# croci/bluest

Measured on AMD Instinct MI355X. Metric: Phi-assemblies/s, higher is better.
Workload: dtype f64; 1 GPU; n=20 models, groups up to size 5 (K_tot=21699), n_out=8, Wishart covariances; one step = V and grad V of one allocation for all outputs; n_models=20, k_max=5, K_tot=21699, n_out=8, batch=1, parallelism=single GPU, evaluation=stored group inverses, launch=hipGraph replay of 20-step graphs (20 of 20 steps), rest eager

## Files before the change

### bluest_amd/build.py

```python
import os
import shutil
import subprocess
import sys

HERE = os.path.dirname(os.path.abspath(__file__))
ROOT = os.path.dirname(HERE)
CSRC = os.path.join(HERE, "csrc")
SOURCES = ["runtime.hip", "mirrors.hip", "plan.hip", "spg.hip", "intproj.hip", "xchg.hip", "newton.hip", "matfree.hip", "mfmc.hip", "mlmc.hip", "covproj.hip", "pilot.hip", "gsums.hip", "fields.hip", "moments.hip", "pilot4.hip", "field_moments.hip", "wave_probe.hip"]
HEADERS = ["common.hpp", "solve.hpp", "plan.hpp", "spg_state.hpp", "jacobi.hpp", "subset_search.hpp", "staging.hpp"]
OBJDIR = os.path.join(CSRC, "_build")
HDR = os.path.join(ROOT, "include", "bluest_hip.h")
LIB = os.path.join(HERE, "libbluest_hip.so")
ARCH = "gfx950"


def hipcc():
    for cand in (os.environ.get("HIPCC"), shutil.which("hipcc"), "/opt/rocm/bin/hipcc"):
        if cand and os.path.exists(cand):
            return cand
    raise RuntimeError("hipcc not found (looked at $HIPCC, PATH, /opt/rocm/bin/hipcc)")


def _inputs():
    return [os.path.join(CSRC, f) for f in SOURCES + HEADERS] + [HDR]


STAMP = os.path.join(OBJDIR, "hipcc_flags.txt")


def _extra_flags():
    return os.environ.get("BLUEST_EXTRA_HIPCC_FLAGS", "").split()


def up_to_date():
    if not os.path.exists(LIB) or os.path.getmtime(LIB) < max(os.path.getmtime(f) for f in _inputs()):
        return False
    try:
        built_with = open(STAMP).read().split()
    except OSError:
        built_with = []
    return built_with == _extra_flags()


SHIM_SRC = os.path.join(HERE, "csrc", "cmisc_shim.cpp")


def shim_path():
    import sysconfig
    return os.path.join(HERE, "shim", "_cmisc_bluest" + sysconfig.get_config_var("EXT_SUFFIX"))


def build_shim(force=False, verbose=False):
    out = shim_path()
    if not force and os.path.exists(out) and os.path.getmtime(out) >= max(os.path.getmtime(SHIM_SRC), os.path.getmtime(HDR)):
        return out
    import pybind11
    import sysconfig
    os.makedirs(os.path.dirname(out), exist_ok=True)
    cmd = ["g++", "-O2", "-shared", "-std=c++17", "-fPIC", "-I" + pybind11.get_include(), "-I" + sysconfig.get_paths()["include"],
           "-I" + os.path.join(ROOT, "include"), SHIM_SRC, "-o", out, "-L" + HERE, "-lbluest_hip", "-Wl,-rpath,$ORIGIN/.."]
    if verbose:
        print(" ".join(cmd))
    subprocess.check_call(cmd)
    return out


def build(force=False, verbose=False):
    if not force and up_to_date():
        build_shim(force=False, verbose=verbose)
        return LIB
    from concurrent.futures import ThreadPoolExecutor
    os.makedirs(OBJDIR, exist_ok=True)
    flags = ["--offload-arch=" + ARCH, "-O3", "-std=c++17", "-fPIC", "-pthread", "-I" + os.path.join(ROOT, "include"),
             "-I" + CSRC] + _extra_flags()

    def compile_one(name):
        obj = os.path.join(OBJDIR, os.path.splitext(name)[0] + ".o")
        cmd = [hipcc()] + flags + ["-c", os.path.join(CSRC, name), "-o", obj]
        if verbose:
            print(" ".join(cmd))
        subprocess.check_call(cmd)
        return obj

    with ThreadPoolExecutor(max_workers=min(len(SOURCES), os.cpu_count() or 1)) as pool:
        objs = list(pool.map(compile_one, SOURCES))
    cmd = [hipcc(), "--offload-arch=" + ARCH, "-shared", "-fPIC", "-pthread", "-o", LIB] + objs
    if verbose:
        print(" ".join(cmd))
    subprocess.check_call(cmd)
    with open(STAMP, "w") as f:
        f.write(" ".join(_extra_flags()))
    build_shim(force=True, verbose=verbose)
    return LIB


if __name__ == "__main__":
    print(build(force="--force" in sys.argv, verbose=True))
```

### bluest_amd/csrc/plan.hip

```cpp

#include "common.hpp"

static int g_debug_timing = getenv("BLUEST_DEBUG_TIMING") ? 1 : 0;
struct PhaseTimer {
    std::chrono::steady_clock::time_point t0 = std::chrono::steady_clock::now();
    const char *what;
    explicit PhaseTimer(const char *w) : what(w) {}
    void lap(const char *phase)
    {
        if (!g_debug_timing) return;
        const auto t1 = std::chrono::steady_clock::now();
        fprintf(stderr, "[bluest timing] %s: %s %.3f ms\n", what, phase, std::chrono::duration<double, std::milli>(t1 - t0).count());
        t0 = t1;
    }
};


#include "plan.hpp"
#include "spg_state.hpp"

template <typename COLT> __device__ __forceinline__ int4 load_cols4(const COLT *p);
template <> __device__ __forceinline__ int4 load_cols4<int32_t>(const int32_t *p) { return *reinterpret_cast<const int4 *>(p); }
template <> __device__ __forceinline__ int4 load_cols4<uint16_t>(const uint16_t *p)
{
    const uint2 w = *reinterpret_cast<const uint2 *>(p);
    return make_int4((int)(w.x & 0xffffu), (int)(w.x >> 16), (int)(w.y & 0xffffu), (int)(w.y >> 16));
}
__device__ __forceinline__ bool phi_gate_closed(const int32_t *gate) { return gate && uniform_word(gate) == 0; }
template <int WPB> __device__ __forceinline__ uint32_t phi_wave_chunk()
{
    if constexpr (WPB == 1) return blockIdx.x;
    else return blockIdx.x * WPB + (uint32_t)__builtin_amdgcn_readfirstlane((int)(threadIdx.x >> 6));
}
template <int WPB, typename COLT>
__global__ __launch_bounds__(64 * WPB) void k_phi_chunks(const double *__restrict__ vals, const COLT *__restrict__ cols,
                                                    int iters, int64_t n_chunks, const double *__restrict__ m,
                                                    int64_t m_stride, int n_cand, double2 *__restrict__ partial,
                                                    const int32_t *__restrict__ pslot, int64_t pstride,
                                                    const int32_t *__restrict__ gate)
{
    kernarg_now(vals, cols, iters, n_chunks, m, m_stride, n_cand, partial, pslot, pstride, gate);
    const bool closed = phi_gate_closed(gate);
    const uint32_t chunk = phi_wave_chunk<WPB>();
    const uint32_t lane = threadIdx.x & 63;
    if (closed) return;
    if (chunk >= (uint32_t)n_chunks) return;
    const int32_t slot_ld = *(pslot ? pslot + chunk : reinterpret_cast<const int32_t *>(cols));
    const uint64_t base = (uint64_t)chunk * ((uint32_t)iters * 256u);
    const char *vb = reinterpret_cast<const char *>(vals + base);
    const char *cb = reinterpret_cast<const char *>(cols + base);
    const double *mc = m;
    char *pc = reinterpret_cast<char *>(partial);
    for (int c = 0; c < n_cand; c++, mc += m_stride, pc += pstride * (int64_t)sizeof(double2)) {
        double s = 0.0, amax = 0.0;
        uint32_t vo = lane * 32u, co = lane * (uint32_t)(4 * sizeof(COLT));
        int it = 0;
        do {
            const double2 *vp = reinterpret_cast<const double2 *>(vb + vo);
            const double2 v01 = vp[0], v23 = vp[1];
            const int4 cc = load_cols4<COLT>(reinterpret_cast<const COLT *>(cb + co));
            const double m0 = mc[cc.x], m1 = mc[cc.y], m2 = mc[cc.z], m3 = mc[cc.w];
            s = fma(v01.x, m0, s);
            s = fma(v01.y, m1, s);
            s = fma(v23.x, m2, s);
            s = fma(v23.y, m3, s);
            amax = fmax(fmax(amax, fmax(fabs(m0), fabs(m1))), fmax(fabs(m2), fabs(m3)));
            vo += 2048u; co += (uint32_t)(256 * sizeof(COLT));
        } while (++it < iters);
        s = wave_sum_dpp(s);
        amax = wave_max_dpp(amax);
        const uint32_t slot = pslot ? (uint32_t)lane_value_here(slot_ld) : chunk;
        if (lane == 0) *reinterpret_cast<double2 *>(pc + slot * 16u) = make_double2(s, amax);
    }
}

template <int OB, int WPB, typename COLT>
__global__ __launch_bounds__(64 * WPB) void k_phi_chunks_shared(const double *__restrict__ vals, const COLT *__restrict__ cols,
                                                           int iters, int64_t ncpo, int n_out, const double *__restrict__ m,
                                                           int64_t m_stride, int n_cand, int64_t pstride, const int32_t *__restrict__ pslot,
                                                           int slots_per_output, double2 *__restrict__ partial, const int32_t *__restrict__ gate)
{
    kernarg_now(vals, cols, iters, ncpo, n_out, m, m_stride, n_cand, pstride, pslot, slots_per_output, partial, gate);
    const bool closed = phi_gate_closed(gate);
    const uint32_t chunk = phi_wave_chunk<WPB>();
    const uint32_t lane = threadIdx.x & 63;
    const uint32_t o0 = blockIdx.y * OB;
    if (closed) return;
    if (chunk >= (uint32_t)ncpo) return;
    const int32_t slot_ld = *(pslot ? pslot + chunk : reinterpret_cast<const int32_t *>(cols));
    const uint32_t ostride = pslot ? (uint32_t)slots_per_output : (uint32_t)ncpo;
    const uint32_t CH = (uint32_t)iters * 256u;
    const char *cb = reinterpret_cast<const char *>(cols + (uint64_t)chunk * CH);
    const uint64_t per_out = (uint64_t)(uint32_t)ncpo * CH;
    const char *vb[OB];
    vb[0] = reinterpret_cast<const char *>(vals + (uint64_t)(o0 * (uint32_t)ncpo + chunk) * CH);
#pragma unroll
    for (int oo = 1; oo < OB; oo++) vb[oo] = vb[oo - 1] + (o0 + oo < (uint32_t)n_out ? per_out * sizeof(double) : 0);
    constexpr int NR = wave_sum_multi_regs(OB);
    uint32_t po[NR];
    bool mine[NR];
#pragma unroll
    for (int j = 0; j < NR; j++) {
        const uint32_t o = o0 + wave_sum_multi_index<OB>(lane, j);
        mine[j] = wave_sum_multi_owner<OB>(lane) && o < (uint32_t)n_out;
        po[j] = o * ostride * 16u;
    }
    const double *mc = m;
    char *pc = reinterpret_cast<char *>(partial);
    for (int c = 0; c < n_cand; c++, mc += m_stride, pc += pstride * (int64_t)sizeof(double2)) {
        double s[OB];
#pragma unroll
        for (int oo = 0; oo < OB; oo++) s[oo] = 0.0;
        double amax = 0.0;
        uint32_t vo = lane * 32u, co = lane * (uint32_t)(4 * sizeof(COLT));
        int it = 0;
        do {
            const int4 cc = load_cols4<COLT>(reinterpret_cast<const COLT *>(cb + co));
            double2 v01[OB], v23[OB];
#pragma unroll
            for (int oo = 0; oo < OB; oo++) {
                const double2 *vp = reinterpret_cast<const double2 *>(vb[oo] + vo);
                v01[oo] = vp[0];
                v23[oo] = vp[1];
            }
            const double m0 = mc[cc.x], m1 = mc[cc.y], m2 = mc[cc.z], m3 = mc[cc.w];
            amax = fmax(fmax(amax, fmax(fabs(m0), fabs(m1))), fmax(fabs(m2), fabs(m3)));
#pragma unroll
            for (int oo = 0; oo < OB; oo++) {
                s[oo] = fma(v01[oo].x, m0, s[oo]);
                s[oo] = fma(v01[oo].y, m1, s[oo]);
                s[oo] = fma(v23[oo].x, m2, s[oo]);
                s[oo] = fma(v23[oo].y, m3, s[oo]);
            }
            vo += 2048u; co += (uint32_t)(256 * sizeof(COLT));
        } while (++it < iters);
        amax = wave_max_dpp(amax);
        double t[NR];
        wave_sum_multi<OB>(s, t);
        const uint32_t slot = pslot ? (uint32_t)lane_value_here(slot_ld) : chunk;
#pragma unroll
        for (int j = 0; j < NR; j++)
            if (mine[j]) *reinterpret_cast<double2 *>(pc + (po[j] + slot * 16u)) = make_double2(t[j], amax);
    }
}

__device__ __forceinline__ bool gate_closed(const int32_t *gate, int *s_closed)
{
    if (!gate) return false;
    if (threadIdx.x == 0) *s_closed = __hip_atomic_load(gate, __ATOMIC_RELAXED, __HIP_MEMORY_SCOPE_AGENT) == 0 ? 1 : 0;
    __syncthreads();
    return *s_closed != 0;
}

template <int NT>
__global__ __launch_bounds__(fold_threads(NT)) void k_solve_from_chunks(int N, int n_out, const RowDesc *__restrict__ rows, int nsym, FoldReg reg,
                                                           const double2 *__restrict__ partial, int64_t n_chunks,
                                                           double delta, int want_v, double *__restrict__ var,
                                                           double *__restrict__ v, int32_t *__restrict__ status,
                                                           const int32_t *__restrict__ gate, double *__restrict__ spg_state, int last_slot, int32_t *__restrict__ spg_enable,
                                                           unsigned int *__restrict__ ticket)
{
    __shared__ SolveLds<NT> lds;
    __shared__ double spg_ls[SPG_STATE_DOUBLES];
    __shared__ int s_closed;
    kernarg_now(N, n_out, rows, nsym, reg.Cd, reg.Co, reg.rank_ab, partial, n_chunks, gate, spg_state);
    const int o = blockIdx.x, c = blockIdx.y, tid = threadIdx.x;
    if (gate_closed(gate, &s_closed)) {
        if (spg_state && tid < WAVE && spg_closed_last(ticket + 16, gridDim.x * gridDim.y, tid))
            spg_decide_wave(spg_state, var, status, n_out, last_slot, spg_enable, spg_ls, tid);
        return;
    }
    SpgPrefetch pf;
    if (spg_state && tid < WAVE) spg_prefetch_state(spg_state, tid, pf);
    if (N < NT) { clear_pads(lds, N, tid, fold_threads(NT)); __syncthreads(); }
    fold_rows(lds, N, rows, o, nsym, partial + (int64_t)c * n_chunks, tid, fold_threads(NT), reg);
    __syncthreads();
    if (tid >= WAVE) return;
    const int lane = tid;
    if (spg_state) spg_prefetch_parts(pf, lane);
    const int64_t e = (int64_t)c * n_out + o;
    if (want_v & 2) {
        if (lane == 0) { var[e] = lds.at(0, 0); status[e] = 0; }
        return;
    }
    const double am = (lane < N) ? lds.amax[lane] : 0.0;
    const bool big = __ballot(am >= 0.05) != 0ull;
    const int reps = (want_v & 4) ? 2 : 1;
    double V_mine = 0.0;
    int32_t st_mine = 0;
    for (int rep = 0; rep < reps; rep++)
        solve_wave<NT>(lds, N, delta, am > 1.0e-6, am > 0.0, big, (want_v & 1) != 0, &V_mine, v + e * N, &st_mine, lane);
    if (lane == 0) { var[e] = V_mine; status[e] = st_mine; }
    if (spg_state) {
        int last = 0;
        if (n_out == 1) {
// ... 125 lines not shown
            const int sh = pow2_exponent(wave_max(rmax));
            if (lane < N)
                for (int j = 0; j < N; j++) A[lane * LD + j] = ldexp(A[lane * LD + j], -sh);
            wave_lds_sync();
            jacobi_pinv_lds(A, Q, N, LD, lane);
            const double w = lane < N ? A[lane * LD + lane] : 0.0;
            const double cut = 1.0e-15 * wave_max(fabs(w));
            if (lane < N) A[lane * LD + lane] = fabs(w) > cut ? 1.0 / w : 0.0;
            wave_lds_sync();
            const int t = __ffsll((long long)mask1) - 1;
            if (pass == 0) {
                double acc = 0.0;
                for (int ee = 0; ee < N; ee++) acc += Q[t * LD + ee] * A[ee * LD + ee] * Q[t * LD + ee];
                V = ldexp(acc, -sh);
            }
            if (pass == npass - 1) {
                double acc = 0.0;
                if (lane < N && (mask2 & 1ull))
                    for (int ee = 0; ee < N; ee++) acc += Q[0 * LD + ee] * A[ee * LD + ee] * Q[lane * LD + ee];
                vmine = ldexp(acc, -sh);
            }
            wave_lds_sync();
        }
    }
    if (lane < N) v[e * N + lane] = vmine;
    if (lane == 0) { var[e] = V; status[e] = st; }
}

template <int KU>
__global__ __launch_bounds__(256) void k_grad_tiles(const TileDesc *__restrict__ tiles, int64_t n_tiles,
                                                    const double *__restrict__ tvals, const double *__restrict__ v,
                                                    const int32_t *__restrict__ status, int N, int n_out, int n_cand,
                                                    double *__restrict__ grad, int64_t grad_stride,
                                                    const int32_t *__restrict__ gate)
{
    if (gate && *gate == 0) return;
    const int64_t t = (int64_t)blockIdx.x * 4 + (threadIdx.x >> 6);
    const int lane = threadIdx.x & 63;
    if (t >= n_tiles) return;
    const TileDesc td = tiles[t];
#define GT(KK) case KK: if (KK <= KU) { grad_tile<(KK <= KU ? KK : 1)>(td, tvals, v, status, N, n_out, n_cand, grad, grad_stride, lane); break; }
    switch (td.k) {
        GT(1) GT(2) GT(3) GT(4) GT(5) GT(6) GT(7) GT(8) GT(9) GT(10) GT(11) GT(12)
        default: grad_tile_generic(td, tvals, v, status, N, n_out, n_cand, grad, grad_stride, lane);
    }
#undef GT
}

__host__ __device__ constexpr int fused_tpb(int NT, int KU) { return (NT <= 26 && KU <= 8) ? 15 : 7; }
using SolveGradKuSet = InstSet<5, 6, 8, 12>;
using GradTilesKuSet = InstSet<5, 8, 12>;
using PhiObSet = InstSet<2, 4, 8>;
template <class F> static void solve_grad_ku_dispatch(int kmax, F &&launch) { SolveGradKuSet::dispatch(kmax, launch); }
template <int NT, int KU>
__global__ __launch_bounds__(64 * (fused_tpb(NT, KU) + 1)) void k_solve_grad(int N, int n_out, const RowDesc *__restrict__ rows, int nsym, FoldReg reg,
                                                    const double2 *__restrict__ partial, const double *__restrict__ rec, double delta,
                                                    const TileDesc *__restrict__ tiles, int64_t n_tiles, int bpo, int tpb, int tile_nt,
                                                    const double *__restrict__ tvals,
                                                    double *__restrict__ var, double *__restrict__ v_ws,
                                                    int32_t *__restrict__ status, double *__restrict__ grad,
                                                    const int32_t *__restrict__ gate, double *__restrict__ spg_state, int last_slot,
                                                    int32_t *__restrict__ spg_enable, unsigned int *__restrict__ ticket, const MaTail ma)
{
    constexpr int FUSED_TPB = fused_tpb(NT, KU);
    constexpr int NTHREADS = 64 * (FUSED_TPB + 1);
    constexpr int PU = tile_pairs(KU);
    __shared__ SolveLds<NT> lds;
    __shared__ double spg_ls[SPG_STATE_DOUBLES];
    kernarg_now(N, n_out, rows, nsym, reg.Cd, reg.Co, reg.rank_ab, partial, rec, tiles, bpo, tpb, gate, spg_state, delta, var, v_ws, status);
    const int tid = threadIdx.x, lane = tid & 63;
    const int wave = __builtin_amdgcn_readfirstlane(tid >> 6);
    int o, first, wg;
    if (bpo > 0) { o = blockIdx.y; first = blockIdx.x == 0; wg = o * bpo + blockIdx.x; }
    else { wg = blockIdx.x; const TileDesc td0 = tile_desc_uniform(tiles, (int64_t)wg * tpb); o = td0.out; first = (td0.n_valid >> 30) & 1; }
    const int64_t t0 = (int64_t)wg * tpb;
    __shared__ int s_closed;
    if (gate_closed(gate, &s_closed)) {
        if (spg_state && first && wave == 0 && spg_closed_last(ticket + 16, (unsigned int)n_out, lane))
            spg_decide_wave(spg_state, var, status, n_out, last_slot, spg_enable, spg_ls, lane);
        return;
    }
    SpgPrefetch pf;
    if (spg_state && first && wave == 0) spg_prefetch_state(spg_state, lane, pf);
    if (N < NT) { clear_pads(lds, N, tid, NTHREADS); __syncthreads(); }
    const double *rec_o = rec ? rec + (int64_t)o * (N * N + 2 * N + 1) : nullptr;
    if (rec_o) {
        for (int t = tid; t < N * N; t += NTHREADS) lds.at(t / N, t % N) = rec_o[t];
    } else {
        fold_rows<NT>(lds, N, rows, o, nsym, partial, tid, NTHREADS, reg);
    }
    TileDesc td;
    td.k = 1; td.n_valid = 0; td.val_off = td.grad_off = 0; td.out = (int16_t)o;
    if (wave > 0 && wave <= tpb) td = tile_desc_uniform(tiles, t0 + wave - 1);
    __syncthreads();
    const int k = td.k;
    double2 pr[PU];
    double V_pub = 0.0;
    int32_t st_pub = 0;
    if (wave == 0) {
        if (spg_state && first) spg_prefetch_parts(pf, lane);
        bool s1, s2, big;
        if (rec_o) {
            s1 = lane < N && rec_o[N * N + lane] > 0.0;
            s2 = lane < N && rec_o[N * N + N + lane] > 0.0;
            big = rec_o[N * N + 2 * N] > 0.0;
        } else {
            const double am = (lane < N) ? lds.amax[lane] : 0.0;
            s1 = am > 1.0e-6;
            s2 = am > 0.0;
            big = __ballot(am >= 0.05) != 0ull;
        }
        double V = 0.0;
        int32_t st = 0;
        solve_wave<NT>(lds, N, delta, s1, s2, big, true, &V, lds.vout, &st, lane);
        if (lane == 0) { lds.status = st; if (ma.x) lds.scratch[0] = V; }
        V_pub = V; st_pub = st;
        if (first) {
            if (lane == 0) { var[o] = V; status[o] = st; }
            if (lane < N) v_ws[(int64_t)o * N + lane] = lds.vout[lane];
        }
    } else if (k <= KU) {
        if (tile_nt) tile_load<PU, true>(pr, tvals + td.val_off, lane, tile_pairs(k));
        else tile_load(pr, tvals + td.val_off, lane, tile_pairs(k));
    }
    __syncthreads();
    if (wave == 0) {
        if (spg_state && first) {
            int last = 0;
            if (n_out == 1) {
                spg_decide_wave(spg_state, var, status, n_out, last_slot, spg_enable, spg_ls, lane, pf, true, V_pub, st_pub);
                return;
            }
            if (lane == 0) {
                asm volatile("s_waitcnt vmcnt(0)" ::: "memory");
                __builtin_amdgcn_fence(__ATOMIC_RELEASE, "agent");
                asm volatile("s_waitcnt vmcnt(0)" ::: "memory");
                const unsigned int t = __hip_atomic_fetch_add(ticket, 1u, __ATOMIC_RELAXED, __HIP_MEMORY_SCOPE_AGENT);
                last = (t == (unsigned int)(n_out - 1)) ? 1 : 0;
                if (last) __hip_atomic_store(ticket, 0u, __ATOMIC_RELAXED, __HIP_MEMORY_SCOPE_AGENT);
            }
            last = __builtin_amdgcn_readfirstlane(last);
            if (last) {
                __builtin_amdgcn_fence(__ATOMIC_ACQUIRE, "agent");
// ... 688 lines not shown
    for (int o = 0; o < lay.n_struct; o++)
        HIP_TRY(hipMemcpy(plan->d_cols + ocb[o] * CH, lay.cols.data() + ss[o], (size_t)(ss[o + 1] - ss[o]) * sizeof(int32_t), hipMemcpyHostToDevice));
    if ((rc = upload(arena, o_rows, &plan->d_rows, lay.rows))) return rc;
    if ((rc = upload(arena, o_tiles, &plan->d_tiles, lay.tiles))) return rc;
    if ((rc = upload(arena, o_invmap, &plan->d_invmap, lay.invmap))) return rc;
    if ((rc = upload(arena, o_goff, &plan->d_goff, plan->grad_off))) return rc;
    if ((rc = upload(arena, o_perm, &lay.d_perm, lay.perm))) return rc;
    if ((rc = upload(arena, o_pslot, &plan->d_pslot, lay.pslot))) return rc;
    if (lay.pslot.empty()) plan->d_pslot = nullptr;
    uint16_t *d_rank_ab = nullptr;
    if ((rc = upload(arena, o_rankab, &d_rank_ab, lay.rank_ab))) return rc;
    plan->fold_reg.rank_ab = lay.rank_ab.empty() ? nullptr : d_rank_ab;
    return BLUEST_OK;
}

static int scatter_values(bluest_plan_t plan, const PlanLayout &lay)
{
    for (int o = 0; o < (int)plan->outs.size(); o++) {
        const OutputDesc &od = plan->outs[o];
        const int st = plan->shared ? 0 : o;
        int64_t io = 0, go = 0, eo = 0;
        for (int k = 1; k <= od.K; k++) {
            const int64_t Lk = od.sizes[k - 1];
            const int ne = k * (k + 1) / 2;
            if (Lk > 0) {
                hipLaunchKernelGGL(k_fill_csr, dim3((unsigned)((Lk * ne + 255) / 256)), dim3(256), 0, 0, od.d_invcov + io, k, Lk,
                                   lay.d_perm + lay.struct_entries[st] + eo, plan->d_vals + lay.out_chunk_begin[o] * lay.CH);
                hipLaunchKernelGGL(k_fill_tiles, dim3((unsigned)((Lk * (ne + k) + 255) / 256)), dim3(256), 0, 0, od.d_invcov + io,
                                   od.d_groups + go, k, Lk, plan->d_tvals + lay.bucket_val[o][k]);
            }
            io += Lk * k * k; go += Lk * k; eo += Lk * ne;
        }
    }
    HIP_TRY(hipGetLastError());
    HIP_TRY(hipStreamSynchronize(0));
    if (plan->fold_reg.Cd > 0) {
        HIP_TRY(hipMemsetAsync(plan->d_partial, 0, (size_t)plan->max_cand * plan->partial_stride * sizeof(double2), 0));
        HIP_TRY(hipStreamSynchronize(0));
    }
    HIP_TRY(hipMemset(plan->d_ticket, 0, 256));
    return BLUEST_OK;
}

extern "C" int bluest_plan_finalize(bluest_plan_t plan, int max_candidates)
{
    if (!plan) return fail(BLUEST_ERR_ARG, "plan is NULL");
    if (plan->finalized) return fail(BLUEST_ERR_STATE, "plan already finalized");
    if (plan->outs.empty()) return fail(BLUEST_ERR_STATE, "plan has no outputs");
    if (max_candidates <= 0 || max_candidates > 65535) return fail(BLUEST_ERR_ARG, "max_candidates=%d out of range", max_candidates);
    const int N = plan->N, n_out = (int)plan->outs.size();
    PhaseTimer timer("plan_finalize");

    plan->nsym = N * (N + 1) / 2;
    plan->max_cand = max_candidates;
    plan->shared = true;
    for (int o = 1; o < n_out; o++) {
        const OutputDesc &x = plan->outs[0], &y = plan->outs[o];
        if (x.K != y.K || x.sizes != y.sizes || x.groups != y.groups || x.mapping != y.mapping) { plan->shared = false; break; }
    }
    PlanLayout lay(n_out, plan->nsym, plan->shared ? 1 : n_out);
    int rc;
    if ((rc = layout_tiles(plan, lay))) return rc;
    plan->identity = plan->shared && plan->outs[0].L_o == plan->L;
    for (int64_t li = 0; plan->identity && li < plan->L; li++) plan->identity = plan->outs[0].mapping[li] == li;
    if ((rc = layout_phi(plan, lay, timer))) return rc;
    layout_fold_reg(plan, lay);
    timer.lap("CSR slots + columns");
    layout_invmap(plan, lay);
    plan->cols16 = plan->L <= 65536 && getenv("BLUEST_COLS32") == nullptr;
    plan->phi_ob_forced = 0;
    if (const char *e = getenv("BLUEST_PHI_OB")) { const int v = atoi(e); if (v == 2 || v == 4 || v == 8) plan->phi_ob_forced = v; }
    plan->phi_bytes = plan->n_chunks * lay.CH * 8 + (plan->shared ? plan->n_chunks / n_out : plan->n_chunks) * lay.CH * (plan->cols16 ? 2 : 4) + plan->n_chunks * 16;
    plan->grad_bytes = (int64_t)lay.n_tvals * 8 + plan->grad_len * 8;
    const char *nt_env = getenv("BLUEST_TILE_NT");
    plan->tile_nt = nt_env ? atoi(nt_env) != 0 : true;
    timer.lap("tile descriptors + inverse maps");
    if ((rc = arena_upload(plan, lay))) return rc;
    timer.lap("device arena + small uploads");
    if ((rc = scatter_values(plan, lay))) return rc;
    plan->finalized = true;
    if ((rc = mf_finalize(plan))) return rc;

    timer.lap("device scatter of the values");
    return BLUEST_OK;
}

int plan_ready(bluest_plan_t plan, int n_cand)
{
    if (!plan) return fail(BLUEST_ERR_ARG, "plan is NULL");
    if (!plan->finalized) return fail(BLUEST_ERR_STATE, "plan not finalized");
    if (n_cand <= 0 || n_cand > plan->max_cand) return fail(BLUEST_ERR_ARG, "n_cand=%d outside 1..%d", n_cand, plan->max_cand);
    return BLUEST_OK;
}

extern "C" int bluest_plan_output_layout(bluest_plan_t plan, int output, int *K, int64_t *sizes, int64_t *mapping)
{
    if (!plan || !K) return fail(BLUEST_ERR_ARG, "null pointer");
    if (output < 0 || output >= (int)plan->outs.size()) return fail(BLUEST_ERR_ARG, "output %d out of range", output);
    const OutputDesc &od = plan->outs[output];
    *K = od.K;
    if (sizes) std::copy(od.sizes.begin(), od.sizes.end(), sizes);
    if (mapping) std::copy(od.mapping.begin(), od.mapping.end(), mapping);
    return BLUEST_OK;
}

extern "C" int bluest_plan_restrict(bluest_plan_t parent, const int64_t *keep, int64_t n_keep, int max_candidates, bluest_plan_t *restricted)
// ... 83 lines not shown
    *n = (int)plan->outs.size();
    return BLUEST_OK;
}

extern "C" int bluest_plan_grad_layout(bluest_plan_t plan, int64_t *grad_len, int64_t *offsets)
{
    if (!plan) return fail(BLUEST_ERR_ARG, "plan is NULL");
    if (!plan->finalized) return fail(BLUEST_ERR_STATE, "plan not finalized");
    if (grad_len) *grad_len = plan->grad_len;
    if (offsets) for (size_t o = 0; o < plan->outs.size(); o++) offsets[o] = plan->grad_off[o];
    return BLUEST_OK;
}

extern "C" int bluest_plan_traffic(bluest_plan_t plan, int64_t *phi_bytes, int64_t *grad_bytes)
{
    if (!plan) return fail(BLUEST_ERR_ARG, "plan is NULL");
    if (!plan->finalized) return fail(BLUEST_ERR_STATE, "plan not finalized");
    if (phi_bytes) *phi_bytes = plan->phi_bytes;
    if (grad_bytes) *grad_bytes = plan->grad_bytes;
    return BLUEST_OK;
}

extern "C" int bluest_plan_phi_len(bluest_plan_t plan, int64_t *len)
{
    if (!plan || !len) return fail(BLUEST_ERR_ARG, "null pointer");
    *len = (int64_t)plan->outs.size() * (plan->N * plan->N + 2 * plan->N + 1);
    return BLUEST_OK;
}

static void launch_grad(bluest_plan_t plan, const double *v_dev, const int32_t *status_dev, int n_cand, double *grad_dev,
                        int64_t grad_stride, hipStream_t st)
{
    GradTilesKuSet::dispatch(plan->kmax, [&](auto ku) {
        hipLaunchKernelGGL((k_grad_tiles<decltype(ku)::value>), dim3((unsigned)((plan->n_tiles + 3) / 4)), dim3(256), 0, st, plan->d_tiles,
                           plan->n_tiles, plan->d_tvals, v_dev, status_dev, plan->N, (int)plan->outs.size(), n_cand, grad_dev, grad_stride, plan->gate);
    });
}

static void launch_solve_from_record(bluest_plan_t plan, const double *rec, int n_cand, double delta, int want_v, double *var_dev,
                                     double *v_dev, int32_t *status_dev, hipStream_t st)
{
    const int n_out = (int)plan->outs.size();
    nt_dispatch(plan->N, [&](auto nt) {
        hipLaunchKernelGGL((k_solve_from_record<decltype(nt)::value>), dim3(n_out, n_cand), dim3(64), 0, st, plan->N, n_out, rec, delta, want_v,
                           var_dev, v_dev, status_dev);
    });
}

static void launch_solve_grad(bluest_plan_t plan, const double *rec, double delta, double *var_dev, int32_t *status_dev, double *grad_dev,
                              double *dec_state, int dec_last, int32_t *dec_enable, MaTail ma, hipStream_t st)
{
    const int n_out = (int)plan->outs.size();
    const dim3 grid = plan->fused_bpo > 0 ? dim3((unsigned)plan->fused_bpo, (unsigned)n_out) : dim3((unsigned)(plan->n_tiles / plan->fused_tpb));
    nt_dispatch(plan->N, [&](auto nt) { solve_grad_ku_dispatch(plan->kmax, [&](auto ku) {
        constexpr int NT = decltype(nt)::value, KU = decltype(ku)::value;
        hipLaunchKernelGGL((k_solve_grad<NT, KU>), grid, dim3(64 * (fused_tpb(NT, KU) + 1)), 0, st, plan->N, n_out, plan->d_rows, plan->nsym,
                           plan->fold_reg, plan->d_partial, rec, delta, plan->d_tiles, plan->n_tiles, plan->fused_bpo, plan->fused_tpb, plan->tile_nt,
                           plan->d_tvals, var_dev, plan->d_v, status_dev, grad_dev, plan->gate, dec_state, dec_last, dec_enable, plan->d_ticket, ma);
    }); });
}

static const int64_t PHI_MIN_WAVES = 2304;
static int phi_ob(const bluest_plan_s *p, int n_cand)
{
    (void)n_cand;
    const int n_out = (int)p->outs.size();
    if (!p->shared || n_out < 2) return 0;
    if (p->phi_ob_forced) return p->phi_ob_forced;
    const int64_t ncpo = p->n_chunks / n_out;
    for (int i = PhiObSet::count - 1; i > 0; i--) {
        const int ob = PhiObSet::values[i];
        if (ob <= n_out && ncpo * ((n_out + ob - 1) / ob) >= PHI_MIN_WAVES) return ob;
    }
    return PhiObSet::values[0];
}

static void launch_chunks(bluest_plan_t p, const double *m, int n_cand, int64_t m_stride, hipStream_t st)
{
    const int n_out = (int)p->outs.size();
    if (const int ob = phi_ob(p, n_cand)) {
        const int64_t ncpo = p->n_chunks / n_out;
        PhiObSet::dispatch(ob, [&](auto obc) {
            constexpr int OB = decltype(obc)::value;
#define LCS2(COLT) hipLaunchKernelGGL((k_phi_chunks_shared<OB, 1, COLT>), dim3((unsigned)ncpo, (n_out + OB - 1) / OB), dim3(64), 0, st, \
                                   p->d_vals, reinterpret_cast<const COLT *>(p->d_cols), p->iters, ncpo, n_out, m, m_stride, n_cand, p->partial_stride, p->d_pslot, p->slots_per_output, p->d_partial, p->gate)
            if (p->cols16) LCS2(uint16_t); else LCS2(int32_t);
#undef LCS2
        });
        return;
    }
#define LPC(COLT) hipLaunchKernelGGL((k_phi_chunks<1, COLT>), dim3((unsigned)p->n_chunks), dim3(64), 0, st, p->d_vals, \
                                  reinterpret_cast<const COLT *>(p->d_cols), p->iters, p->n_chunks, m, m_stride, n_cand, p->d_partial, p->d_pslot, p->partial_stride, p->gate)
    if (p->cols16) LPC(uint16_t); else LPC(int32_t);
#undef LPC
}

extern "C" int bluest_plan_phi_chunks(bluest_plan_t plan, const double *m_dev, int n_cand, int64_t m_stride, void *stream)
{
    int rc = plan_ready(plan, n_cand); if (rc) return rc;
    if (!m_dev) return fail(BLUEST_ERR_ARG, "null pointer");
    if (n_cand > 1 && m_stride < plan->L) return fail(BLUEST_ERR_ARG, "m_stride < L_global");
    launch_chunks(plan, m_dev, n_cand, m_stride, (hipStream_t)stream);
    HIP_TRY(hipGetLastError());
    return BLUEST_OK;
}

extern "C" int bluest_plan_phi(bluest_plan_t plan, const double *m_dev, int n_cand, int64_t m_stride, double *phi_dev, void *stream)
{
    int rc = plan_ready(plan, n_cand); if (rc) return rc;
    if (!m_dev || !phi_dev) return fail(BLUEST_ERR_ARG, "null pointer");
    if (n_cand > 1 && m_stride < plan->L) return fail(BLUEST_ERR_ARG, "m_stride < L_global");
    hipStream_t st = (hipStream_t)stream;
    const int n_out = (int)plan->outs.size();
    if (plan->matfree && n_cand == 1 && !plan->gate) return mf_phi_record(plan, m_dev, phi_dev, nullptr, st);
    launch_chunks(plan, m_dev, n_cand, m_stride, st);
    nt_dispatch(plan->N, [&](auto nt) {
        hipLaunchKernelGGL((k_fold_to_record<decltype(nt)::value>), dim3(n_out, n_cand), dim3(fold_threads(nt)), 0, st, plan->N, n_out, plan->d_rows,
                           plan->nsym, plan->fold_reg, plan->d_partial, plan->partial_stride, phi_dev);
    });
    HIP_TRY(hipGetLastError());
    return BLUEST_OK;
}

extern "C" int bluest_plan_solve(bluest_plan_t plan, const double *phi_dev, int n_cand, double delta, double *var_dev,
                                 double *v_dev, int32_t *status_dev, void *stream)
{
    int rc = plan_ready(plan, n_cand); if (rc) return rc;
    if (!phi_dev || !var_dev || !v_dev || !status_dev) return fail(BLUEST_ERR_ARG, "null pointer");
    launch_solve_from_record(plan, phi_dev, n_cand, delta, 1, var_dev, v_dev, status_dev, (hipStream_t)stream);
    HIP_TRY(hipGetLastError());
    return BLUEST_OK;
}

extern "C" int bluest_plan_solve_pinv(bluest_plan_t plan, const double *phi_dev, int n_cand, double delta, double *var_dev,
                                      double *v_dev, int32_t *status_dev, void *stream)
{
    int rc = plan_ready(plan, n_cand); if (rc) return rc;
    if (!phi_dev || !var_dev || !v_dev || !status_dev) return fail(BLUEST_ERR_ARG, "null pointer");
    const int n_out = (int)plan->outs.size(), N = plan->N;
    const size_t lds = (size_t)2 * N * (N + 1) * sizeof(double);
    if (lds > (48u << 10)) (void)hipFuncSetAttribute((const void *)k_pinv_from_record, hipFuncAttributeMaxDynamicSharedMemorySize, (int)lds);
    hipLaunchKernelGGL(k_pinv_from_record, dim3(n_out, n_cand), dim3(64), lds, (hipStream_t)stream, N, n_out, phi_dev, delta, var_dev,
                       v_dev, status_dev);
    HIP_TRY(hipGetLastError());
    return BLUEST_OK;
// ... 195 lines not shown
```

### bluest_amd/csrc/solve.hpp

```cpp
#pragma once
#include "common.hpp"

struct RowDesc {
    int32_t first_chunk;
    int32_t n_chunks;
    int16_t out, a, b, pad;
};


template <int NT>
struct SolveLds {
    static constexpr int LDP = NT + 2;
    double phi[NT * LDP];
    double amax[NT];
    double vout[NT];
    double scratch[NT <= 32 && NT > 16 ? 16 * (NT - 15) : 1];
    int status;
    __device__ __forceinline__ double &at(int a, int b) { return phi[(NT - 1 - a) * LDP + (NT - 1 - b)]; }
};

template <int NT>
__device__ __forceinline__ void clear_pads(SolveLds<NT> &lds, int N, int tid, int nthreads)
{
    if (N < NT)
        for (int t = tid; t < NT * SolveLds<NT>::LDP; t += nthreads) lds.phi[t] = 0.0;
}

__device__ __forceinline__ double readlane_f64(double x, int l)
{
    const int lo = __builtin_amdgcn_readlane(__double2loint(x), l);
    const int hi = __builtin_amdgcn_readlane(__double2hiint(x), l);
    return __hiloint2double(hi, lo);
}

template <int CTRL>
__device__ __forceinline__ double dpp_f64(double x)
{
    const int lo = __builtin_amdgcn_mov_dpp(__double2loint(x), CTRL, 0xf, 0xf, true);
    const int hi = __builtin_amdgcn_mov_dpp(__double2hiint(x), CTRL, 0xf, 0xf, true);
    return __hiloint2double(hi, lo);
}
__device__ __forceinline__ double row_sum(double v)
{
    v += dpp_f64<0xB1>(v);
    v += dpp_f64<0x4E>(v);
    v += dpp_f64<0x141>(v);
    v += dpp_f64<0x140>(v);
    return v;
}
__device__ __forceinline__ double fast_sum(double v)
{
    v = row_sum(v);
    return (readlane_f64(v, 0) + readlane_f64(v, 16)) + (readlane_f64(v, 32) + readlane_f64(v, 48));
}
__device__ __forceinline__ double fast_max(double v)
{
    v = fmax(v, dpp_f64<0xB1>(v));
    v = fmax(v, dpp_f64<0x4E>(v));
    v = fmax(v, dpp_f64<0x141>(v));
    v = fmax(v, dpp_f64<0x140>(v));
    return fmax(fmax(readlane_f64(v, 0), readlane_f64(v, 16)), fmax(readlane_f64(v, 32), readlane_f64(v, 48)));
}
__device__ __forceinline__ double opaque_zero()
{
    double z;
    asm("v_mov_b64 %0, 0" : "=v"(z));
    return z;
}
struct FoldReg { int Cd, Co; const uint16_t *rank_ab; };
template <int NT>
__device__ __forceinline__ void fold_rows(SolveLds<NT> &lds, int N, const RowDesc *__restrict__ rows, int o,
                                          int n_rows, const double2 *__restrict__ partial, int tid, int nthreads, FoldReg reg)
{
    const int q = tid & 3;
    if (reg.Cd > 0) {
        const int slots = N * reg.Cd + (n_rows - N) * reg.Co;
        const double2 *po = partial + (int64_t)o * slots;
        for (int r = tid >> 2; r < n_rows; r += nthreads >> 2) {
            const bool dg = r < N;
            const int n = dg ? reg.Cd : reg.Co;
            const double2 *p = po + (dg ? r * reg.Cd : N * reg.Cd + (r - N) * reg.Co);
            const unsigned ab = reg.rank_ab[r];
            double s = opaque_zero(), am = opaque_zero();
            for (int c0 = q; c0 < n; c0 += 32) {
                double2 v[8];
#pragma unroll
                for (int i = 0; i < 8; i++) v[i] = (c0 + 4 * i < n) ? p[c0 + 4 * i] : make_double2(0.0, 0.0);
#pragma unroll
                for (int i = 0; i < 8; i++) { s += v[i].x; am = fmax(am, v[i].y); }
            }
            const int a = (int)(ab & 0xffu), b = (int)(ab >> 8);
            s += quad_x1(s);
            am = fmax(am, quad_x1(am));
            s += quad_x2(s);
            am = fmax(am, quad_x2(am));
            if (q == 0) {
                lds.at(a, b) = s;
                lds.at(b, a) = s;
                if (dg) lds.amax[a] = am;
            }
        }
        return;
    }
    for (int r = tid >> 2; r < n_rows; r += nthreads >> 2) {
        const RowDesc rd = rows[o * n_rows + r];
        const double2 *p = partial + rd.first_chunk;
        const int n = rd.n_chunks;
        double s = opaque_zero(), am = opaque_zero();
        for (int c0 = q; c0 < n; c0 += 32) {
            double2 v[8];
#pragma unroll
            for (int i = 0; i < 8; i++) v[i] = (c0 + 4 * i < n) ? p[c0 + 4 * i] : make_double2(0.0, 0.0);
#pragma unroll
            for (int i = 0; i < 8; i++) { s += v[i].x; am = fmax(am, v[i].y); }
        }
        s += quad_x1(s);
        am = fmax(am, quad_x1(am));
        s += quad_x2(s);
        am = fmax(am, quad_x2(am));
        if (q == 0) {
            lds.at(rd.a, rd.b) = s;
            lds.at(rd.b, rd.a) = s;
            if (rd.a == rd.b) lds.amax[rd.a] = am;
        }
    }
}

__device__ __forceinline__ int uniform_i(int x) { return __builtin_amdgcn_readfirstlane(x); }

__device__ __forceinline__ double rcp_f64(double x)
{
    double y = __builtin_amdgcn_rcp(x);
    double e = fma(-x, y, 1.0);
    y = fma(y, e, y);
    e = fma(-x, y, 1.0);
    y = fma(y, e, y);
    return y;
}

#define BLUEST_PIVOT_TOL 1.0e-14
template <int NT>
__device__ __forceinline__ void gj_regs(double (&a)[NT], int lane, double diag0, double &rinv_mine, double &last_pivot, int &bad)
{
    const double floor_mine = BLUEST_PIVOT_TOL * diag0;
    bool flag = false;
#pragma unroll
    for (int j = 0; j < NT; j++) {
        const double piv = readlane_f64(a[j], j);
        const bool is = lane == j;
        flag = is ? !(a[j] > floor_mine) : flag;
        const double rinv = rcp_f64(piv);
        rinv_mine = is ? rinv : rinv_mine;
        if (j == NT - 1) { last_pivot = piv; break; }
        const double f = is ? 0.0 : -a[j] * rinv;
        double u[NT];
#pragma unroll
        for (int c = j + 1; c < NT; c++) u[c] = readlane_f64(a[c], j);
#pragma unroll
        for (int c = j + 1; c < NT; c++) a[c] = fma(f, u[c], a[c]);
    }
    bad |= (__ballot(flag && lane < NT) != 0ull || !isfinite(last_pivot)) ? 1 : 0;
}

template <int NT> struct GjMap {
    static constexpr bool dpp = NT <= 32;
// ... 240 lines not shown
```

Measured before the change: 785,600 assemblies/s (one output: Phi(m) over all groups -> V, grad V).

## Preload kernargs into SGPRs and reorder/pack arguments for phi and solve kernels

Compiles plan.hip with kernarg preloading and reorders the phi-chunk and fused solve-grad kernel arguments so the ones needed first sit at the front. N and nsym are packed into one word, and optional pointers are replaced by a flags word. Late-needed arguments are loaded only after the first memory loads are issued, which is meant to hide the kernarg fetch latency at kernel start. This relies on an LLVM option and adds a limit of N <= 64 to fit the packed argument.

```diff
diff --git a/bluest_amd/build.py b/bluest_amd/build.py
--- a/bluest_amd/build.py
+++ b/bluest_amd/build.py
@@ -8,6 +8,7 @@
 CSRC = os.path.join(HERE, "csrc")
 SOURCES = ["runtime.hip", "mirrors.hip", "plan.hip", "spg.hip", "intproj.hip", "xchg.hip", "newton.hip", "matfree.hip", "mfmc.hip", "mlmc.hip", "covproj.hip", "pilot.hip", "gsums.hip", "fields.hip", "moments.hip", "pilot4.hip", "field_moments.hip", "wave_probe.hip"]
 HEADERS = ["common.hpp", "solve.hpp", "plan.hpp", "spg_state.hpp", "jacobi.hpp", "subset_search.hpp", "staging.hpp"]
+SOURCE_FLAGS = {"plan.hip": ["-mllvm", "-amdgpu-kernarg-preload-count=16"]}
 OBJDIR = os.path.join(CSRC, "_build")
 HDR = os.path.join(ROOT, "include", "bluest_hip.h")
 LIB = os.path.join(HERE, "libbluest_hip.so")
@@ -32,14 +33,18 @@
     return os.environ.get("BLUEST_EXTRA_HIPCC_FLAGS", "").split()
 
 
+def _stamp_text():
+    return "\n".join([" ".join(_extra_flags())] + ["%s: %s" % (name, " ".join(SOURCE_FLAGS[name])) for name in sorted(SOURCE_FLAGS)])
+
+
 def up_to_date():
     if not os.path.exists(LIB) or os.path.getmtime(LIB) < max(os.path.getmtime(f) for f in _inputs()):
         return False
     try:
-        built_with = open(STAMP).read().split()
+        built_with = open(STAMP).read()
     except OSError:
-        built_with = []
-    return built_with == _extra_flags()
+        built_with = None
+    return built_with == _stamp_text()
 
 
 SHIM_SRC = os.path.join(HERE, "csrc", "cmisc_shim.cpp")
@@ -72,11 +77,11 @@
     from concurrent.futures import ThreadPoolExecutor
     os.makedirs(OBJDIR, exist_ok=True)
     flags = ["--offload-arch=" + ARCH, "-O3", "-std=c++17", "-fPIC", "-pthread", "-I" + os.path.join(ROOT, "include"),
-             "-I" + CSRC] + _extra_flags()
+             "-I" + CSRC]
 
     def compile_one(name):
         obj = os.path.join(OBJDIR, os.path.splitext(name)[0] + ".o")
-        cmd = [hipcc()] + flags + ["-c", os.path.join(CSRC, name), "-o", obj]
+        cmd = [hipcc()] + flags + SOURCE_FLAGS.get(name, []) + _extra_flags() + ["-c", os.path.join(CSRC, name), "-o", obj]
         if verbose:
             print(" ".join(cmd))
         subprocess.check_call(cmd)
@@ -89,7 +94,7 @@
         print(" ".join(cmd))
     subprocess.check_call(cmd)
     with open(STAMP, "w") as f:
-        f.write(" ".join(_extra_flags()))
+        f.write(_stamp_text())
     build_shim(force=True, verbose=verbose)
     return LIB
 
diff --git a/bluest_amd/csrc/plan.hip b/bluest_amd/csrc/plan.hip
--- a/bluest_amd/csrc/plan.hip
+++ b/bluest_amd/csrc/plan.hip
@@ -26,32 +26,32 @@
     const uint2 w = *reinterpret_cast<const uint2 *>(p);
     return make_int4((int)(w.x & 0xffffu), (int)(w.x >> 16), (int)(w.y & 0xffffu), (int)(w.y >> 16));
 }
-__device__ __forceinline__ bool phi_gate_closed(const int32_t *gate) { return gate && uniform_word(gate) == 0; }
 template <int WPB> __device__ __forceinline__ uint32_t phi_wave_chunk()
 {
     if constexpr (WPB == 1) return blockIdx.x;
     else return blockIdx.x * WPB + (uint32_t)__builtin_amdgcn_readfirstlane((int)(threadIdx.x >> 6));
 }
+constexpr uint32_t PHI_HAS_GATE = 1u;
+template <class... A> __device__ __forceinline__ void phi_late_args(const A &...a) { kernarg_now(a...); }
 template <int WPB, typename COLT>
 __global__ __launch_bounds__(64 * WPB) void k_phi_chunks(const double *__restrict__ vals, const COLT *__restrict__ cols,
-                                                    int iters, int64_t n_chunks, const double *__restrict__ m,
-                                                    int64_t m_stride, int n_cand, double2 *__restrict__ partial,
-                                                    const int32_t *__restrict__ pslot, int64_t pstride,
-                                                    const int32_t *__restrict__ gate)
-{
-    kernarg_now(vals, cols, iters, n_chunks, m, m_stride, n_cand, partial, pslot, pstride, gate);
-    const bool closed = phi_gate_closed(gate);
+                                                    const double *__restrict__ m, const int32_t *__restrict__ pslot,
+                                                    int iters, uint32_t n_chunks, int n_out, int n_cand, uint32_t flags,
+                                                    const int32_t *__restrict__ gate, int64_t m_stride, int64_t pstride,
+                                                    int slots_per_output, double2 *__restrict__ partial)
+{
+    (void)n_out; (void)slots_per_output;
     const uint32_t chunk = phi_wave_chunk<WPB>();
     const uint32_t lane = threadIdx.x & 63;
-    if (closed) return;
-    if (chunk >= (uint32_t)n_chunks) return;
-    const int32_t slot_ld = *(pslot ? pslot + chunk : reinterpret_cast<const int32_t *>(cols));
+    if (flags & PHI_HAS_GATE) { if (uniform_word(gate) == 0) return; }
+    if (chunk >= n_chunks) return;
+    const int32_t slot_ld = uniform_word(pslot ? pslot + chunk : reinterpret_cast<const int32_t *>(cols));
     const uint64_t base = (uint64_t)chunk * ((uint32_t)iters * 256u);
     const char *vb = reinterpret_cast<const char *>(vals + base);
     const char *cb = reinterpret_cast<const char *>(cols + base);
     const double *mc = m;
-    char *pc = reinterpret_cast<char *>(partial);
-    for (int c = 0; c < n_cand; c++, mc += m_stride, pc += pstride * (int64_t)sizeof(double2)) {
+    int64_t pdone = 0;
+    for (int c = 0; c < n_cand; c++) {
         double s = 0.0, amax = 0.0;
         uint32_t vo = lane * 32u, co = lane * (uint32_t)(4 * sizeof(COLT));
         int it = 0;
@@ -59,6 +59,7 @@
             const double2 *vp = reinterpret_cast<const double2 *>(vb + vo);
             const double2 v01 = vp[0], v23 = vp[1];
             const int4 cc = load_cols4<COLT>(reinterpret_cast<const COLT *>(cb + co));
+            phi_late_args(m_stride, pstride, partial);
             const double m0 = mc[cc.x], m1 = mc[cc.y], m2 = mc[cc.z], m3 = mc[cc.w];
             s = fma(v01.x, m0, s);
             s = fma(v01.y, m1, s);
@@ -69,45 +70,45 @@
         } while (++it < iters);
         s = wave_sum_dpp(s);
         amax = wave_max_dpp(amax);
-        const uint32_t slot = pslot ? (uint32_t)lane_value_here(slot_ld) : chunk;
+        const uint32_t slot = pslot ? (uint32_t)uniform_value_here(slot_ld) : chunk;
+        char *pc = reinterpret_cast<char *>(uniform_value_here(partial)) + pdone;
         if (lane == 0) *reinterpret_cast<double2 *>(pc + slot * 16u) = make_double2(s, amax);
+        mc += uniform_value_here(m_stride);
+        pdone += uniform_value_here(pstride) * (int64_t)sizeof(double2);
     }
 }
 
 template <int OB, int WPB, typename COLT>
 __global__ __launch_bounds__(64 * WPB) void k_phi_chunks_shared(const double *__restrict__ vals, const COLT *__restrict__ cols,
-                                                           int iters, int64_t ncpo, int n_out, const double *__restrict__ m,
-                                                           int64_t m_stride, int n_cand, int64_t pstride, const int32_t *__restrict__ pslot,
-                                                           int slots_per_output, double2 *__restrict__ partial, const int32_t *__restrict__ gate)
-{
-    kernarg_now(vals, cols, iters, ncpo, n_out, m, m_stride, n_cand, pstride, pslot, slots_per_output, partial, gate);
-    const bool closed = phi_gate_closed(gate);
+                                                           const double *__restrict__ m, const int32_t *__restrict__ pslot,
+                                                           int iters, uint32_t ncpo, int n_out, int n_cand, uint32_t flags,
+                                                           const int32_t *__restrict__ gate, int64_t m_stride, int64_t pstride,
+                                                           int slots_per_output, double2 *__restrict__ partial)
+{
     const uint32_t chunk = phi_wave_chunk<WPB>();
     const uint32_t lane = threadIdx.x & 63;
     const uint32_t o0 = blockIdx.y * OB;
-    if (closed) return;
-    if (chunk >= (uint32_t)ncpo) return;
-    const int32_t slot_ld = *(pslot ? pslot + chunk : reinterpret_cast<const int32_t *>(cols));
-    const uint32_t ostride = pslot ? (uint32_t)slots_per_output : (uint32_t)ncpo;
+    if (flags & PHI_HAS_GATE) { if (uniform_word(gate) == 0) return; }
+    if (chunk >= ncpo) return;
+    const int32_t slot_ld = uniform_word(pslot ? pslot + chunk : reinterpret_cast<const int32_t *>(cols));
     const uint32_t CH = (uint32_t)iters * 256u;
     const char *cb = reinterpret_cast<const char *>(cols + (uint64_t)chunk * CH);
-    const uint64_t per_out = (uint64_t)(uint32_t)ncpo * CH;
+    const uint64_t per_out = (uint64_t)ncpo * CH;
     const char *vb[OB];
-    vb[0] = reinterpret_cast<const char *>(vals + (uint64_t)(o0 * (uint32_t)ncpo + chunk) * CH);
+    vb[0] = reinterpret_cast<const char *>(vals + (uint64_t)(o0 * ncpo + chunk) * CH);
 #pragma unroll
     for (int oo = 1; oo < OB; oo++) vb[oo] = vb[oo - 1] + (o0 + oo < (uint32_t)n_out ? per_out * sizeof(double) : 0);
     constexpr int NR = wave_sum_multi_regs(OB);
-    uint32_t po[NR];
+    uint32_t on[NR];
     bool mine[NR];
 #pragma unroll
     for (int j = 0; j < NR; j++) {
-        const uint32_t o = o0 + wave_sum_multi_index<OB>(lane, j);
-        mine[j] = wave_sum_multi_owner<OB>(lane) && o < (uint32_t)n_out;
-        po[j] = o * ostride * 16u;
+        on[j] = o0 + wave_sum_multi_index<OB>(lane, j);
+        mine[j] = wave_sum_multi_owner<OB>(lane) && on[j] < (uint32_t)n_out;
     }
     const double *mc = m;
-    char *pc = reinterpret_cast<char *>(partial);
-    for (int c = 0; c < n_cand; c++, mc += m_stride, pc += pstride * (int64_t)sizeof(double2)) {
+    int64_t pdone = 0;
+    for (int c = 0; c < n_cand; c++) {
         double s[OB];
 #pragma unroll
         for (int oo = 0; oo < OB; oo++) s[oo] = 0.0;
@@ -122,6 +123,7 @@
                 const double2 *vp = reinterpret_cast<const double2 *>(vb[oo] + vo);
                 v01[oo] = vp[0];
                 v23[oo] = vp[1];
+                if (oo == (OB < 4 ? OB : 4) - 1) phi_late_args(m_stride, pstride, slots_per_output, partial);
             }
             const double m0 = mc[cc.x], m1 = mc[cc.y], m2 = mc[cc.z], m3 = mc[cc.w];
             amax = fmax(fmax(amax, fmax(fabs(m0), fabs(m1))), fmax(fabs(m2), fabs(m3)));
@@ -134,13 +136,17 @@
             }
             vo += 2048u; co += (uint32_t)(256 * sizeof(COLT));
         } while (++it < iters);
-        amax = wave_max_dpp(amax);
         double t[NR];
         wave_sum_multi<OB>(s, t);
-        const uint32_t slot = pslot ? (uint32_t)lane_value_here(slot_ld) : chunk;
+        amax = wave_max_dpp(amax);
+        const uint32_t slot = pslot ? (uint32_t)uniform_value_here(slot_ld) : chunk;
+        const uint32_t ostride = pslot ? (uint32_t)uniform_value_here(slots_per_output) : ncpo;
+        char *pc = reinterpret_cast<char *>(uniform_value_here(partial)) + pdone;
 #pragma unroll
         for (int j = 0; j < NR; j++)
-            if (mine[j]) *reinterpret_cast<double2 *>(pc + (po[j] + slot * 16u)) = make_double2(t[j], amax);
+            if (mine[j]) *reinterpret_cast<double2 *>(pc + (on[j] * ostride + slot) * 16u) = make_double2(t[j], amax);
+        mc += uniform_value_here(m_stride);
+        pdone += uniform_value_here(pstride) * (int64_t)sizeof(double2);
     }
 }
 
@@ -372,14 +378,16 @@
 using GradTilesKuSet = InstSet<5, 8, 12>;
 using PhiObSet = InstSet<2, 4, 8>;
 template <class F> static void solve_grad_ku_dispatch(int kmax, F &&launch) { SolveGradKuSet::dispatch(kmax, launch); }
+constexpr uint32_t SG_HAS_REC = 1u, SG_HAS_GATE = 2u, SG_HAS_SPG = 4u;
 template <int NT, int KU>
-__global__ __launch_bounds__(64 * (fused_tpb(NT, KU) + 1)) void k_solve_grad(int N, int n_out, const RowDesc *__restrict__ rows, int nsym, FoldReg reg,
-                                                    const double2 *__restrict__ partial, const double *__restrict__ rec, double delta,
-                                                    const TileDesc *__restrict__ tiles, int64_t n_tiles, int bpo, int tpb, int tile_nt,
+__global__ __launch_bounds__(64 * (fused_tpb(NT, KU) + 1)) void k_solve_grad(const double2 *__restrict__ partial, const uint16_t *__restrict__ rank_ab,
+                                                    const RowDesc *__restrict__ rows, const TileDesc *__restrict__ tiles,
+                                                    uint32_t n_nsym, int Cd, int Co, int bpo, uint32_t flags,
+                                                    int n_out_arg, int tpb_arg, int tile_nt, const double *__restrict__ rec_arg, double delta,
                                                     const double *__restrict__ tvals,
                                                     double *__restrict__ var, double *__restrict__ v_ws,
                                                     int32_t *__restrict__ status, double *__restrict__ grad,
-                                                    const int32_t *__restrict__ gate, double *__restrict__ spg_state, int last_slot,
+                                                    const int32_t *__restrict__ gate, double *__restrict__ spg_state_arg, int last_slot,
                                                     int32_t *__restrict__ spg_enable, unsigned int *__restrict__ ticket, const MaTail ma)
 {
     constexpr int FUSED_TPB = fused_tpb(NT, KU);
@@ -387,28 +395,35 @@
     constexpr int PU = tile_pairs(KU);
     __shared__ SolveLds<NT> lds;
     __shared__ double spg_ls[SPG_STATE_DOUBLES];
-    kernarg_now(N, n_out, rows, nsym, reg.Cd, reg.Co, reg.rank_ab, partial, rec, tiles, bpo, tpb, gate, spg_state, delta, var, v_ws, status);
+    const int N = (int)(n_nsym & 0xffu), nsym = (int)(n_nsym >> 8);
+    const FoldReg reg{Cd, Co, rank_ab};
     const int tid = threadIdx.x, lane = tid & 63;
     const int wave = __builtin_amdgcn_readfirstlane(tid >> 6);
     int o, first, wg;
     if (bpo > 0) { o = blockIdx.y; first = blockIdx.x == 0; wg = o * bpo + blockIdx.x; }
-    else { wg = blockIdx.x; const TileDesc td0 = tile_desc_uniform(tiles, (int64_t)wg * tpb); o = td0.out; first = (td0.n_valid >> 30) & 1; }
-    const int64_t t0 = (int64_t)wg * tpb;
+    else { wg = blockIdx.x; const TileDesc td0 = tile_desc_uniform(tiles, (int64_t)wg * tpb_arg); o = td0.out; first = (td0.n_valid >> 30) & 1; }
     __shared__ int s_closed;
-    if (gate_closed(gate, &s_closed)) {
-        if (spg_state && first && wave == 0 && spg_closed_last(ticket + 16, (unsigned int)n_out, lane))
-            spg_decide_wave(spg_state, var, status, n_out, last_slot, spg_enable, spg_ls, lane);
-        return;
+    double *spg_state = nullptr;
+    if (flags & (SG_HAS_GATE | SG_HAS_SPG)) {
+        if (flags & SG_HAS_SPG) spg_state = spg_state_arg;
+        if ((flags & SG_HAS_GATE) && gate_closed(gate, &s_closed)) {
+            if (spg_state && first && wave == 0 && spg_closed_last(ticket + 16, (unsigned int)n_out_arg, lane))
+                spg_decide_wave(spg_state, var, status, n_out_arg, last_slot, spg_enable, spg_ls, lane);
+            return;
+        }
     }
     SpgPrefetch pf;
     if (spg_state && first && wave == 0) spg_prefetch_state(spg_state, lane, pf);
     if (N < NT) { clear_pads(lds, N, tid, NTHREADS); __syncthreads(); }
-    const double *rec_o = rec ? rec + (int64_t)o * (N * N + 2 * N + 1) : nullptr;
+    const double *rec_o = (flags & SG_HAS_REC) ? rec_arg + (int64_t)o * (N * N + 2 * N + 1) : nullptr;
     if (rec_o) {
         for (int t = tid; t < N * N; t += NTHREADS) lds.at(t / N, t % N) = rec_o[t];
     } else {
-        fold_rows<NT>(lds, N, rows, o, nsym, partial, tid, NTHREADS, reg);
-    }
+        fold_rows<NT>(lds, N, rows, o, nsym, partial, tid, NTHREADS, reg,
+                      [&]() { kernarg_now(n_out_arg, tpb_arg, delta, var, v_ws, status); });
+    }
+    const int n_out = uniform_value_here(n_out_arg), tpb = uniform_value_here(tpb_arg);
+    const int64_t t0 = (int64_t)wg * tpb;
     TileDesc td;
     td.k = 1; td.n_valid = 0; td.val_off = td.grad_off = 0; td.out = (int16_t)o;
     if (wave > 0 && wave <= tpb) td = tile_desc_uniform(tiles, t0 + wave - 1);
@@ -1203,6 +1218,7 @@
     PhaseTimer timer("plan_finalize");
 
     plan->nsym = N * (N + 1) / 2;
+    if (N > 64 || plan->nsym > 2080) return fail(BLUEST_ERR_ARG, "N=%d: the fused kernel's argument word holds N <= 64, nsym <= 2080", N);
     plan->max_cand = max_candidates;
     plan->shared = true;
     for (int o = 1; o < n_out; o++) {
@@ -1392,11 +1408,13 @@
 {
     const int n_out = (int)plan->outs.size();
     const dim3 grid = plan->fused_bpo > 0 ? dim3((unsigned)plan->fused_bpo, (unsigned)n_out) : dim3((unsigned)(plan->n_tiles / plan->fused_tpb));
+    const uint32_t flags = (rec ? SG_HAS_REC : 0u) | (plan->gate ? SG_HAS_GATE : 0u) | (dec_state ? SG_HAS_SPG : 0u);
     nt_dispatch(plan->N, [&](auto nt) { solve_grad_ku_dispatch(plan->kmax, [&](auto ku) {
         constexpr int NT = decltype(nt)::value, KU = decltype(ku)::value;
-        hipLaunchKernelGGL((k_solve_grad<NT, KU>), grid, dim3(64 * (fused_tpb(NT, KU) + 1)), 0, st, plan->N, n_out, plan->d_rows, plan->nsym,
-                           plan->fold_reg, plan->d_partial, rec, delta, plan->d_tiles, plan->n_tiles, plan->fused_bpo, plan->fused_tpb, plan->tile_nt,
-                           plan->d_tvals, var_dev, plan->d_v, status_dev, grad_dev, plan->gate, dec_state, dec_last, dec_enable, plan->d_ticket, ma);
+        hipLaunchKernelGGL((k_solve_grad<NT, KU>), grid, dim3(64 * (fused_tpb(NT, KU) + 1)), 0, st, plan->d_partial, plan->fold_reg.rank_ab, plan->d_rows,
+                           plan->d_tiles, (uint32_t)plan->N | (uint32_t)plan->nsym << 8, plan->fold_reg.Cd, plan->fold_reg.Co, plan->fused_bpo, flags,
+                           n_out, plan->fused_tpb, (int)plan->tile_nt, rec, delta, plan->d_tvals, var_dev, plan->d_v, status_dev, grad_dev,
+                           plan->gate, dec_state, dec_last, dec_enable, plan->d_ticket, ma);
     }); });
 }
 
@@ -1418,19 +1436,22 @@
 static void launch_chunks(bluest_plan_t p, const double *m, int n_cand, int64_t m_stride, hipStream_t st)
 {
     const int n_out = (int)p->outs.size();
+    const uint32_t flags = p->gate ? PHI_HAS_GATE : 0u;
     if (const int ob = phi_ob(p, n_cand)) {
         const int64_t ncpo = p->n_chunks / n_out;
         PhiObSet::dispatch(ob, [&](auto obc) {
             constexpr int OB = decltype(obc)::value;
 #define LCS2(COLT) hipLaunchKernelGGL((k_phi_chunks_shared<OB, 1, COLT>), dim3((unsigned)ncpo, (n_out + OB - 1) / OB), dim3(64), 0, st, \
-                                   p->d_vals, reinterpret_cast<const COLT *>(p->d_cols), p->iters, ncpo, n_out, m, m_stride, n_cand, p->partial_stride, p->d_pslot, p->slots_per_output, p->d_partial, p->gate)
+                                   p->d_vals, reinterpret_cast<const COLT *>(p->d_cols), m, p->d_pslot, p->iters, (uint32_t)ncpo, n_out, n_cand, flags, \
+                                   p->gate, m_stride, p->partial_stride, p->slots_per_output, p->d_partial)
             if (p->cols16) LCS2(uint16_t); else LCS2(int32_t);
 #undef LCS2
         });
         return;
     }
 #define LPC(COLT) hipLaunchKernelGGL((k_phi_chunks<1, COLT>), dim3((unsigned)p->n_chunks), dim3(64), 0, st, p->d_vals, \
-                                  reinterpret_cast<const COLT *>(p->d_cols), p->iters, p->n_chunks, m, m_stride, n_cand, p->d_partial, p->d_pslot, p->partial_stride, p->gate)
+                                  reinterpret_cast<const COLT *>(p->d_cols), m, p->d_pslot, p->iters, (uint32_t)p->n_chunks, n_out, n_cand, flags, \
+                                  p->gate, m_stride, p->partial_stride, p->slots_per_output, p->d_partial)
     if (p->cols16) LPC(uint16_t); else LPC(int32_t);
 #undef LPC
 }
diff --git a/bluest_amd/csrc/solve.hpp b/bluest_amd/csrc/solve.hpp
--- a/bluest_amd/csrc/solve.hpp
+++ b/bluest_amd/csrc/solve.hpp
@@ -68,9 +68,11 @@
     return z;
 }
 struct FoldReg { int Cd, Co; const uint16_t *rank_ab; };
-template <int NT>
+struct FoldNoHook { __device__ __forceinline__ void operator()() const {} };
+template <int NT, class Hook = FoldNoHook>
 __device__ __forceinline__ void fold_rows(SolveLds<NT> &lds, int N, const RowDesc *__restrict__ rows, int o,
-                                          int n_rows, const double2 *__restrict__ partial, int tid, int nthreads, FoldReg reg)
+                                          int n_rows, const double2 *__restrict__ partial, int tid, int nthreads, FoldReg reg,
+                                          const Hook &issued = Hook())
 {
     const int q = tid & 3;
     if (reg.Cd > 0) {
@@ -86,6 +88,7 @@
                 double2 v[8];
 #pragma unroll
                 for (int i = 0; i < 8; i++) v[i] = (c0 + 4 * i < n) ? p[c0 + 4 * i] : make_double2(0.0, 0.0);
+                issued();
 #pragma unroll
                 for (int i = 0; i < 8; i++) { s += v[i].x; am = fmax(am, v[i].y); }
             }
@@ -111,6 +114,7 @@
             double2 v[8];
 #pragma unroll
             for (int i = 0; i < 8; i++) v[i] = (c0 + 4 * i < n) ? p[c0 + 4 * i] : make_double2(0.0, 0.0);
+            issued();
 #pragma unroll
             for (int i = 0; i < 8; i++) { s += v[i].x; am = fmax(am, v[i].y); }
         }
```

After: 813,400 assemblies/s (one output: Phi(m) over all groups -> V, grad V), median of 6. 1.04x the previous value.
